# haoheliu/voicefixer

Hardware: AMD Instinct MI355X
Metric: seconds-of-44.1kHz-audio restored per wall-second (higher is better)
Workload: dtype f32

## Files before the change

include/vfx_hip.h:

```cpp
#ifndef VFX_HIP_H
#define VFX_HIP_H

#include <stddef.h>
#include <stdint.h>

#ifdef __cplusplus
extern "C" {
#endif

typedef void* vfx_stream_t;

#define VFX_OK 0
#define VFX_EINVAL (-1)
#define VFX_EALIGN (-2)
#define VFX_ERANGE (-3)
#define VFX_ENOTSUP (-4)

typedef struct {
    void* ptr;
    int64_t bstride, cstride, lstride;
    int64_t guard;
    const int32_t* rows;
} vfx_tensor;

// ... 22 lines not shown
    const float* w_direct;
    const float* w_wino4;
} vfx_act;

#define VFX_PAD_ZERO 0
#define VFX_PAD_REFLECT 1

int vfx_version(void);

const char* vfx_build_id(void);

uint64_t vfx_launch_count(void);

int vfx_last_conv_tile(void);


int vfx_conv1d_f32(const vfx_tensor* x, const float* w_packed, const float* bias,
                   const vfx_tensor* res, const vfx_tensor* y, int B, int Cin, int Cout, int L,
                   int k, int dilation, int pad_mode, const vfx_act* act, vfx_stream_t stream);

int vfx_conv1d_f16(const vfx_tensor* x, const void* w_f16, const float* bias, const vfx_tensor* res,
                   const vfx_tensor* y, int B, int C, int L, int dilation, const vfx_act* act, int32_t* range_flag,
                   vfx_stream_t stream);

typedef struct {
    const float* w1_direct;
    const float* bias1;
    const float* w2_direct;
    const float* bias2;
    const float* w2_wino;
// ... 147 lines not shown
```

voicefixer_amd/_lib.py:

```python
import ctypes as C
import os
import subprocess

from ._dev import dev_env

_HERE = os.path.dirname(os.path.abspath(__file__))
LIB_PATH = dev_env("VFX_LIB", os.path.join(_HERE, "libvfx_hip.so"))
CSRC = os.path.join(_HERE, "csrc")


class VfxError(RuntimeError):
    pass


class vfx_tensor(C.Structure):
    _fields_ = [("ptr", C.c_void_p), ("bstride", C.c_int64), ("cstride", C.c_int64),
                ("lstride", C.c_int64), ("guard", C.c_int64), ("rows", C.c_void_p)]


class vfx_act(C.Structure):
    _fields_ = [("pre_act", C.c_int), ("pre_slope", C.c_float), ("pre_scale", C.c_void_p),
                ("pre_shift", C.c_void_p), ("post_act", C.c_int), ("post_slope", C.c_float),
                ("math", C.c_int), ("w_x3", C.c_void_p), ("w_direct", C.c_void_p), ("w_wino4", C.c_void_p)]

# ... 7 lines not shown
POST_NONE, POST_LRELU, POST_ELU, POST_TANH, POST_SIGMOID, POST_LRELU_SNAKE = 0, 1, 2, 3, 4, 5
PAD_ZERO, PAD_REFLECT = 0, 1
MATH_F32, MATH_BF16X3 = 0, 1
EINVAL, EALIGN, ERANGE, ENOTSUP = -1, -2, -3, -4

_T = C.POINTER(vfx_tensor)
_A = C.POINTER(vfx_act)
_P = C.c_void_p
_I = C.c_int

SIGNATURES = {
    "vfx_version": (_I, []),
    "vfx_build_id": (C.c_char_p, []),
    "vfx_launch_count": (C.c_uint64, []),
    "vfx_last_conv_tile": (_I, []),
    "vfx_conv1d_f32": (_I, [_T, _P, _P, _T, _T, _I, _I, _I, _I, _I, _I, _I, _A, _P]),
    "vfx_conv1d_f16": (_I, [_T, _P, _P, _T, _T, _I, _I, _I, _I, _A, _P, _P]),
    "vfx_resblock_f32": (_I, [_T, _T, C.POINTER(vfx_resblock_w), _I, _I, _I, _I, C.c_float, _I, C.c_float, _P]),
    "vfx_resblock_wino4_f32": (_I, [_T, _T, C.POINTER(vfx_resblock_w), _I, _I, _I, _I, C.c_float, _I, C.c_float, _P]),
    "vfx_convtr1d_f32": (_I, [_T, _P, _P, _T, _I, _I, _I, _I, _I, _A, _P]),
    "vfx_conv2d_f32": (_I, [_T, _P, _P, _T, _T, _I, _I, _I, _I, _I, _I, _A, _P]),
    "vfx_convtr2d_3x3s2_f32": (_I, [_T, _P, _T, _I, _I, _I, _I, _I, _A, _P]),
    "vfx_conv1d_cout1_f32": (_I, [_T, _P, _P, _T, _I, _I, _I, _I, _I, _I, _I, _P]),
    "vfx_avgpool2x2_f32": (_I, [_T, _T, _I, _I, _I, _I, _P]),
    "vfx_frontend_init": (_I, [_P, _P, _P, _P, _P, _P, _I]),
    "vfx_frontend_readback": (_I, [_I, _P, _P, _P, _P, _I, C.POINTER(_I)]),
    "vfx_stft_mel_f32": (_I, [_P, C.c_int64, _I, _I, _P, _P]),
    "vfx_stft_mel_rows_f32": (_I, [_P, C.c_int64, _I, _P, _I, _P, _P]),
    "vfx_post_rows_f32": (_I, [_P, C.c_int64, _I, _P, _P, C.c_int64, _P, _I, _I, _P, _P]),
    "vfx_mel_to_cond_rows_f32": (_I, [_P, _T, _I, _I, _P, _I, _P]),
# ... 72 lines not shown
```

voicefixer_amd/csrc/vfx_conv.hip:

```cpp
#include "vfx_common.h"
#include <cstdio>
#include <cstdlib>
#include <cstring>
#include <map>
#include <mutex>
#include <string>
#include <type_traits>
#include <vector>

#ifndef VFX_X3_ABL
#define VFX_X3_ABL 0
#endif
#ifndef VFX_ABL
#define VFX_ABL 0
#endif
#define VFX_MAXPH 8
#define VFX_MAXT 9

typedef float f32x16 __attribute__((ext_vector_type(16)));
typedef unsigned int u32x4 __attribute__((ext_vector_type(4)));

#if VFX_ABL & 8
__device__ unsigned long long g_dbg[10];
__device__ unsigned long long g_dbgx[6];
// ... 942 lines not shown
            fprintf(stderr, "conv table:");
            const unsigned* w = reinterpret_cast<const unsigned*>(&tb);
            for (size_t i = 0; i < sizeof(PhaseTab) / 4; ++i) fprintf(stderr, " %08x", w[i]);
            fprintf(stderr, "\n");
        }
    }
    ConvTables* d = nullptr;
    if (hipMalloc((void**)&d, sizeof(ConvTables)) != hipSuccess) return nullptr;
    if (hipMemcpy(d, &tb, sizeof(ConvTables), hipMemcpyHostToDevice) != hipSuccess) return nullptr;
    cache.emplace(std::move(key), d);
    return d;
}

static thread_local int g_last_tile = 0;
extern "C" int vfx_last_conv_tile(void) { return g_last_tile; }

static inline int floor4(int v) { return v >= 0 ? (v & ~3) : -(((-v) + 3) & ~3); }

template <int BM, int BL, int WGM, int WGL, int KC, bool FAST, int NXV = 4, bool SPLITK = false>
static int launch_one(const ConvArgs& a, dim3 grid, size_t lds, hipStream_t s) {
    static unsigned long long attr_set = 0;
    int attr_dev = 0;
    if (hipGetDevice(&attr_dev) != hipSuccess) attr_dev = 0;
    auto kern = conv_taps_kernel<BM, BL, WGM, WGL, KC, FAST, NXV, SPLITK>;
    if (!((attr_set >> (attr_dev & 63)) & 1ull)) {
        hipError_t e = hipFuncSetAttribute(reinterpret_cast<const void*>(kern),
                                           hipFuncAttributeMaxDynamicSharedMemorySize, 160 * 1024);
        if (e != hipSuccess) return (int)e;
        attr_set |= 1ull << (attr_dev & 63);
    }
    {
        static const bool dump = VFX_DEV_ENV("VFX_DEBUG_ARGS") && atoi(VFX_DEV_ENV("VFX_DEBUG_ARGS")) != 0;
        if (dump) {
            fprintf(stderr, "conv_taps<%d,%d,%d,%d,%d,%d,%d,%d> grid %u %u %u lds %zu args:", BM, BL, WGM, WGL, KC, (int)FAST,
                    NXV, (int)SPLITK, grid.x, grid.y, grid.z, lds);
            const unsigned* w = reinterpret_cast<const unsigned*>(&a);
            for (size_t i = 0; i < sizeof(ConvArgs) / 4; ++i) fprintf(stderr, " %08x", w[i]);
            fprintf(stderr, "\n");
        }
    }
    hipLaunchKernelGGL(kern, grid, dim3(64 * WGM * WGL), lds, s, a);
    VFX_LAUNCHED();
    return vfx_last_error();
}

template <int BM, int BL, int WGM, int WGL, int KC>
static int launch_cfg(const ConvArgs& a, int ntiles, int gy, int gz, size_t lds, hipStream_t s) {
    const int nfast = a.tile_hi - a.tile_lo;
    int rc = VFX_OK;
    if (a.ksplit > 1) {
        if (nfast > 0) rc = launch_one<BM, BL, WGM, WGL, KC, true, 4, true>(a, dim3(nfast, gy, gz), lds, s);
        if (rc == VFX_OK && ntiles - nfast > 0)
            rc = launch_one<BM, BL, WGM, WGL, KC, false, 4, true>(a, dim3(ntiles - nfast, gy, gz), lds, s);
        return rc;
    }
    if (nfast > 0) {
        const dim3 grid((nfast + a.tpw - 1) / a.tpw, gy, gz);
// ... 98 lines not shown

template <int BM, int BL, int WGM, int WGL, int NT, int MODE, int ROWS = 1>
static int launch_x3_one(const ConvArgs& a, dim3 grid, size_t lds, hipStream_t s) {
    static unsigned long long attr_set = 0;
    int attr_dev = 0;
    if (hipGetDevice(&attr_dev) != hipSuccess) attr_dev = 0;
    auto kern = conv_x3_kernel<BM, BL, WGM, WGL, NT, MODE, ROWS>;
    if (!((attr_set >> (attr_dev & 63)) & 1ull)) {
        hipError_t e = hipFuncSetAttribute(reinterpret_cast<const void*>(kern),
                                           hipFuncAttributeMaxDynamicSharedMemorySize, 160 * 1024);
        if (e != hipSuccess) return (int)e;
        attr_set |= 1ull << (attr_dev & 63);
    }
    hipLaunchKernelGGL(kern, grid, dim3(256), lds, s, a);
    VFX_LAUNCHED();
    return vfx_last_error();
}

template <int BM, int BL, int WGM, int WGL>
static int launch_x3_tile(const ConvArgs& a, int nt, int mode, int rows, dim3 grid, size_t lds, hipStream_t s) {
    if (rows == 3 && nt == 3) return launch_x3_one<BM, BL, WGM, WGL, 3, 0, 3>(a, grid, lds, s);
    if (rows == 3) return launch_x3_one<BM, BL, WGM, WGL, 1, 0, 3>(a, grid, lds, s);
#define VFX_X3(NT_)                                                                                  \
    if (nt == NT_)                                                                                   \
        return mode == 2   ? launch_x3_one<BM, BL, WGM, WGL, NT_, 2>(a, grid, lds, s)                \
               : mode == 1 ? launch_x3_one<BM, BL, WGM, WGL, NT_, 1>(a, grid, lds, s)                \
                           : launch_x3_one<BM, BL, WGM, WGL, NT_, 0>(a, grid, lds, s);
    VFX_X3(1)
    VFX_X3(2)
    VFX_X3(3)
// ... 411 lines not shown
```

voicefixer_amd/csrc/vfx_convh.inc:

```

typedef _Float16 f16x8 __attribute__((ext_vector_type(8)));
typedef _Float16 f16x2 __attribute__((ext_vector_type(2)));
typedef float f32x2h __attribute__((ext_vector_type(2)));

namespace convh {
constexpr int BM = 128, BL = 128, KC = 32, NTHR = 256;
constexpr int NPMAX = 3 * BL;
constexpr int NU = (KC / 8) * NPMAX / NTHR;
constexpr int BUFB = (KC / 8) * NPMAX * 16;
constexpr float F16_MAX = 65504.f;
}

struct ConvhArgs {
    const float* x; long long x_bs, x_cs;
    const int32_t* x_rows;
    const _Float16* w;
    const float* bias;
    const float* res; long long r_bs, r_cs;
    float* y; long long y_bs, y_cs;
    int C, L, d, ntiles, nm;
    int pre_act; float pre_slope;
    int post_act; float post_slope;
    int32_t* flag;
};
// ... 162 lines not shown
    a.res = res ? static_cast<const float*>(res->ptr) : nullptr;
    a.r_bs = res ? res->bstride : 0; a.r_cs = res ? res->cstride : 0;
    a.y = static_cast<float*>(y->ptr); a.y_bs = y->bstride; a.y_cs = y->cstride;
    a.C = C; a.L = L; a.d = dilation;
    a.ntiles = (L + convh::BL - 1) / convh::BL;
    a.nm = C / convh::BM;
    a.pre_act = pre; a.pre_slope = act ? act->pre_slope : 0.f;
    a.post_act = post; a.post_slope = act ? act->post_slope : 0.f;
    a.flag = range_flag;
    const long long nblk = (long long)a.ntiles * a.nm;
    if (nblk > 0x7fffffffLL) return VFX_ENOTSUP;
    auto kern = bias ? (a.res ? convh_kernel<true, true> : convh_kernel<true, false>)
                     : (a.res ? convh_kernel<false, true> : convh_kernel<false, false>);
    hipLaunchKernelGGL(kern, dim3((unsigned)nblk, 1, B), dim3(convh::NTHR), 0, (hipStream_t)stream, a);
    VFX_LAUNCHED();
    g_last_tile = convh::BM * 100000 + convh::BL * 100 + 32;
    return vfx_last_error();
}
```

voicefixer_amd/csrc/vfx_convtw.inc:

```
template <int WGM, int WGP>
__global__ __launch_bounds__(256, 2) void convtw_kernel(const ConvArgs a) {
    static_assert(WGM * WGP == 4, "four waves");
    constexpr int KC = 16, NSTEP = KC / 2, NPL = 4;
    constexpr int BM = 32 * WGM, BT = 32 * WGP;
    constexpr int CG = 256 / BT;
    constexpr int NSLOT = KC / CG;
    constexpr int SPAN = NSTEP / NSLOT;
    constexpr int PLANE = KC * BT;
    constexpr int BUF = NPL * PLANE;
    extern __shared__ __attribute__((aligned(16))) float smem[];

    const int tid = threadIdx.x, lane = tid & 63;
    const int wave = __builtin_amdgcn_readfirstlane(tid >> 6);
    const int lo = lane & 31, hi = lane >> 5;
    const int wm = wave / WGP, wp = wave % WGP;
    const int s = a.nph_fold, gy = a.tpw;
    int lin = blockIdx.x;
    if (a.xcd_chunk > 0) lin = (lin & 7) * a.xcd_chunk + (lin >> 3);
    if (lin >= a.ntiles_l * gy) return;
    int mblk, tile;
    if (a.tile_lo == 0) {
        tile = lin % a.ntiles_l; mblk = lin / a.ntiles_l;
    } else {
        mblk = lin % gy; tile = lin / gy;
// ... 213 lines not shown
                for (int j = 0; j < 4; ++j) {
                    const bool one = !all4 && o4 + j >= 0 && o4 + j < sL;
                    __builtin_amdgcn_raw_buffer_store_b32(u[j], yrsrc, one ? yb + 4 * j : VFX_W_OOB, 0, 0);
                }
            }
        }
        __builtin_amdgcn_fence(__ATOMIC_ACQ_REL, "wavefront");
        __builtin_amdgcn_wave_barrier();
    }
}

template <int WGM, int WGP>
static int launch_convtw(const ConvArgs& a, dim3 grid, size_t lds, hipStream_t s) {
    hipLaunchKernelGGL((convtw_kernel<WGM, WGP>), grid, dim3(256), lds, s, a);
    VFX_LAUNCHED();
    return vfx_last_error();
}

static int try_launch_convtw(const vfx_tensor* x, const float* w_packed, const float* w32, const float* bias, const vfx_tensor* y, int B,
                             int Cin, int Cout, int Lin, int stride, const vfx_act* act, hipStream_t stream) {
    static const bool off = VFX_DEV_ENV("VFX_CONVTW") && atoi(VFX_DEV_ENV("VFX_CONVTW")) == 0;
    if (off || !w_packed || !w32 || !vfx_aligned16(w32) || !x || !y || !x->ptr || !y->ptr) return VFX_ENOTSUP;
    if (act && (act->pre_act != VFX_PRE_NONE || act->post_act != VFX_POST_NONE || act->math != VFX_MATH_F32)) return VFX_ENOTSUP;
    if (Cin < 32 || Cout <= 0 || Cin % 32 != 0 || Cout % 64 != 0 || B <= 0 || B > 65535 || Lin < 1 || stride < 1) return VFX_ENOTSUP;
    if (x->lstride != 1 || y->lstride != 1 || (bias && !vfx_aligned16(bias))) return VFX_ENOTSUP;
    const long long lim = (1ll << 31) - (1ll << 20);
    if (((long long)Cin * x->cstride + Lin) * 4 >= lim || ((long long)Cout * y->cstride + (long long)stride * Lin) * 4 >= lim) return VFX_ENOTSUP;
    if (4ll * stride * (Cin >> 3) * Cout * 32 >= lim || (long long)stride * stride * Cout >= (1ll << 32)) return VFX_ENOTSUP;
    const bool wide = Cout % 128 == 0;
    const int BT = wide ? 32 : 64;
// ... 30 lines not shown
```

voicefixer_amd/csrc/vfx_convw.inc:

```

#define VFX_W_MAXNT 3
#ifndef VFX_W_MULTITILE
#define VFX_W_MULTITILE 0
#endif

template <int RM>
struct WStream {
    int voff[RM];
    int gstride;
    int cin8;
    int slab0, slab_step;
    int nt;
    int t, c8, c8_last;
    float4 cur[RM], nxt[RM];

    __device__ __forceinline__ void load(__amdgpu_buffer_rsrc_t rsrc, float4 (&dst)[RM]) {
        const int soff = ((slab0 + t * slab_step) * cin8 + c8) * gstride;
#pragma unroll
        for (int i = 0; i < RM; ++i) {
            const u32x4 r = __builtin_amdgcn_raw_buffer_load_b128(rsrc, voff[i], soff, 0);
            dst[i] = make_float4(__uint_as_float(r.x), __uint_as_float(r.y), __uint_as_float(r.z), __uint_as_float(r.w));
        }
        int tn = t + 1, cn = c8;
        if (tn == nt) { tn = 0; cn = c8 + 1; }
// ... 793 lines not shown

template <int BM, int BL, int WGM, int WGL, int NT, int NXV, int FUSED>
static int launch_w_one(const ConvArgs& a, dim3 grid, size_t lds, hipStream_t s) {
    static unsigned long long attr_set = 0;
    int attr_dev = 0;
    if (hipGetDevice(&attr_dev) != hipSuccess) attr_dev = 0;
    auto kern = convw_kernel<BM, BL, WGM, WGL, NT, NXV, FUSED>;
    if (!((attr_set >> (attr_dev & 63)) & 1ull)) {
        hipError_t e = hipFuncSetAttribute(reinterpret_cast<const void*>(kern),
                                           hipFuncAttributeMaxDynamicSharedMemorySize, 160 * 1024);
        if (e != hipSuccess) return (int)e;
        attr_set |= 1ull << (attr_dev & 63);
    }
    hipLaunchKernelGGL(kern, grid, dim3(256), lds, s, a);
    VFX_LAUNCHED();
    return vfx_last_error();
}

template <int BM, int BL, int WGM, int WGL, int NT, int FUSED>
static int launch_w_nxv(const ConvArgs& a, dim3 grid, size_t lds, hipStream_t s) {
    if constexpr (FUSED) {
        return a.nxv <= 5 ? launch_w_one<BM, BL, WGM, WGL, NT, 5, FUSED>(a, grid, lds, s)
                          : launch_w_one<BM, BL, WGM, WGL, NT, 6, FUSED>(a, grid, lds, s);
    } else if constexpr (NT == 9) {
        return a.nxv <= 4 ? launch_w_one<BM, BL, WGM, WGL, NT, 4, false>(a, grid, lds, s)
                          : launch_w_one<BM, BL, WGM, WGL, NT, 7, false>(a, grid, lds, s);
    } else {
        return a.nxv <= 4   ? launch_w_one<BM, BL, WGM, WGL, NT, 4, false>(a, grid, lds, s)
               : a.nxv == 5 ? launch_w_one<BM, BL, WGM, WGL, NT, 5, false>(a, grid, lds, s)
                            : launch_w_one<BM, BL, WGM, WGL, NT, 6, false>(a, grid, lds, s);
// ... 320 lines not shown
```

voicefixer_amd/csrc/vfx_convwg.inc:

```

static void convwg_fold_blocks(ConvArgs& a, dim3& grid, int gy) {
    static const bool off = VFX_DEV_ENV("VFX_WINO_MFOLD") && atoi(VFX_DEV_ENV("VFX_WINO_MFOLD")) == 0;
    a.nph_fold = 0;
    if (gy > 1 && a.xcd_chunk > 0 && !off) {
        a.nph_fold = gy;
        grid = dim3(grid.x * gy, 1, grid.z);
    }
}

#ifndef VFX_WG4_OCC
#define VFX_WG4_OCC 2
#endif
#ifndef VFX_WG4_ABL
#define VFX_WG4_ABL 0
#endif
#ifndef VFX_WG4_SPEC2_OCC
#define VFX_WG4_SPEC2_OCC 2
#endif
template <int WGM, int WGP, bool D1 = false, int XD = 2, bool PRE = true, int SPEC = 0>
__global__ __launch_bounds__(256, (SPEC == 2 && WGM == 4) ? VFX_WG4_SPEC2_OCC : VFX_WG4_OCC) void convwg4_kernel(const ConvArgs a) {
    static_assert(WGM * WGP == 4, "four waves");
    static_assert(SPEC == 0 || (SPEC == 1 && PRE) || (SPEC == 2 && D1 && !PRE), "specialised instances");
    constexpr bool ZSTART = SPEC != 0;
    static_assert(XD == 2 || XD == 3, "prefetch distance");
// ... 494 lines not shown

template <int WGM, int WGP, bool D1 = false, int XD = 2, bool PRE = true, int SPEC = 0>
static int launch_wg4_xd(const ConvArgs& a, dim3 grid, size_t lds, hipStream_t s) {
    static unsigned long long attr_set = 0;
    int attr_dev = 0;
    if (hipGetDevice(&attr_dev) != hipSuccess) attr_dev = 0;
    auto kern = convwg4_kernel<WGM, WGP, D1, XD, PRE, SPEC>;
    if (!((attr_set >> (attr_dev & 63)) & 1ull)) {
        hipError_t e = hipFuncSetAttribute(reinterpret_cast<const void*>(kern),
                                           hipFuncAttributeMaxDynamicSharedMemorySize, 160 * 1024);
        if (e != hipSuccess) return (int)e;
        attr_set |= 1ull << (attr_dev & 63);
    }
    hipLaunchKernelGGL(kern, grid, dim3(256), lds, s, a);
    VFX_LAUNCHED();
    return vfx_last_error();
}

template <int WGM, int WGP, bool D1 = false>
static int launch_wg4_one(const ConvArgs& a, dim3 grid, size_t lds, hipStream_t s) {
#ifdef VFX_DEV
    static const int xd = VFX_DEV_ENV("VFX_WG4_XD") ? atoi(VFX_DEV_ENV("VFX_WG4_XD")) : 2;
    if (xd == 3) return launch_wg4_xd<WGM, WGP, D1, 3, true>(a, grid, lds, s);
    static const int spec_mask = VFX_DEV_ENV("VFX_WG4_SPEC") ? atoi(VFX_DEV_ENV("VFX_WG4_SPEC")) : 3;
#else
    constexpr int spec_mask = 3;
#endif
    if ((spec_mask & 1) && !a.res && a.pre_act == VFX_PRE_LRELU && a.post_act == VFX_POST_LRELU && (!a.bias || vfx_aligned16(a.bias)))
        return launch_wg4_xd<WGM, WGP, D1, 2, true, 1>(a, grid, lds, s);
    if constexpr (D1) {
// ... 84 lines not shown
```

voicefixer_amd/csrc/vfx_convwg2d.inc:

```
constexpr int WG4S_TWO_CIN = 384;
template <int WGM, int WGP, int KC, bool AFF = true, bool TWO = false>
__global__ __launch_bounds__(256, TWO ? 1 : 2) void convwg4s_kernel(const ConvArgs a) {
    static_assert(WGM * WGP == 4 && (KC == 8 || KC == 16), "four waves; 8- or 16-channel chunks");
    constexpr int NSTEP = KC / 2;
    constexpr int NG = KC / 8;
    constexpr int NSEQ = 3 * NG;
    constexpr int BM = 32 * WGM, BQ = 32 * WGP;
    constexpr int ROW = BQ + 2;
    constexpr int CG = 256 / BQ;
    constexpr int NSLOT = KC / CG;
    constexpr int PLANE = KC * ROW;
    constexpr int BUF = 6 * PLANE;
    static_assert(2 * NSLOT <= 3 * NSTEP, "two steps of staging per element must fit the chunk");
    extern __shared__ __attribute__((aligned(16))) float smem[];

    const int tid = threadIdx.x, lane = tid & 63;
    const int wave = __builtin_amdgcn_readfirstlane(tid >> 6);
    const int lo = lane & 31, hi = lane >> 5;
    const int wm = wave / WGP, wp = wave % WGP;
    int bx = blockIdx.x;
    int mblk = blockIdx.y;
    if (a.xcd_chunk > 0) {
        int k = bx >> 3;
        if (a.nph_fold > 1) {
// ... 272 lines not shown
                __builtin_amdgcn_raw_buffer_store_b32(__float_as_uint(keep ? fmaxf(y[i], y[i] * ps) : 0.f), yrsrc, yv[i], soff, 0);
        }
    } else {
#pragma unroll 1
        for (int r = 0; r < 16; ++r) {
            const int soff = (row0 + (r & 3) + 8 * (r >> 2)) * ycs4;
            float y[4];
            outs(r, y);
#pragma unroll
            for (int i = 0; i < 4; ++i)
                __builtin_amdgcn_raw_buffer_store_b32(__float_as_uint(keep ? vfx_post(y[i], post, ps) : 0.f), yrsrc, yv[i], soff, 0);
        }
    }
}

template <int WGM, int WGP, int KC, bool AFF, bool TWO>
static int launch_wg4s_aff(const ConvArgs& a, dim3 grid, size_t lds, hipStream_t s) {
    static unsigned long long attr_set = 0;
    int attr_dev = 0;
    if (hipGetDevice(&attr_dev) != hipSuccess) attr_dev = 0;
    auto kern = convwg4s_kernel<WGM, WGP, KC, AFF, TWO>;
    if (!((attr_set >> (attr_dev & 63)) & 1ull)) {
        hipError_t e = hipFuncSetAttribute(reinterpret_cast<const void*>(kern),
                                           hipFuncAttributeMaxDynamicSharedMemorySize, 160 * 1024);
        if (e != hipSuccess) return (int)e;
        attr_set |= 1ull << (attr_dev & 63);
    }
    hipLaunchKernelGGL(kern, grid, dim3(256), lds, s, a);
    VFX_LAUNCHED();
    return vfx_last_error();
}

template <int WGM, int WGP, int KC>
static int launch_wg4s_one(const ConvArgs& a, dim3 grid, size_t lds, hipStream_t s) {
    if (a.Cin > WG4S_TWO_CIN)
        return a.pre_act == VFX_PRE_NONE ? launch_wg4s_aff<WGM, WGP, KC, false, true>(a, grid, lds, s)
                                         : launch_wg4s_aff<WGM, WGP, KC, true, true>(a, grid, lds, s);
    return a.pre_act == VFX_PRE_NONE ? launch_wg4s_aff<WGM, WGP, KC, false, false>(a, grid, lds, s)
                                     : launch_wg4s_aff<WGM, WGP, KC, true, false>(a, grid, lds, s);
}

static int try_launch_convwg4s_2d(ConvArgs a, const vfx_tensor* x, int P, const float* wg4, hipStream_t stream) {
    static const bool off = (VFX_DEV_ENV("VFX_WINO") && atoi(VFX_DEV_ENV("VFX_WINO")) == 0) ||
                            (VFX_DEV_ENV("VFX_WINO4") && atoi(VFX_DEV_ENV("VFX_WINO4")) == 0) ||
// ... 17 lines not shown
            return VFX_ENOTSUP;
        if (18ll * (a.CinPad >> 3) * a.Cout * 32 >= lim) return VFX_ENOTSUP;
    }
    const int d = P;
    const long long nquads = ((long long)a.Lin + 4 * d - 1) / (4 * d) * d;
    const int ntiles = (int)((nquads + BQ - 1) / BQ);
    const int gy = a.Cout / (narrow ? 32 : 64);
    if ((long long)ntiles * gy * a.B < 384) return VFX_ENOTSUP;
    a.wd = wg4;
    a.wg_d = d;
    a.x_guard = 0;
    a.tab = nullptr;
    a.stagger = 0; a.stagger_wgs = 0;
    if (!a.res) { a.r_bs = a.x_bs; a.r_cs = a.x_cs; }
    const size_t lds = (2ull * 6 * kc * (BQ + 2) + 2ull * a.Cin) * sizeof(float);
    dim3 grid(convw_grid_x(a, ntiles), gy, a.B);
    convwg_fold_blocks(a, grid, gy);
    g_last_tile = (narrow ? 32 : 64) * 100000 + (4 * BQ % 1000) * 100 + 88;
    return narrow ? launch_wg4s_one<1, 4, 8>(a, grid, lds, stream) : launch_wg4s_one<2, 2, 16>(a, grid, lds, stream);
}
```

voicefixer_amd/csrc/vfx_convwg4p.inc:

```
template <int WGM, int WGP, bool D1, bool PRE, int SPEC>
__global__ __launch_bounds__(256, 2) void convwg4p_kernel(const ConvArgs a) {
    static_assert(WGM * WGP == 4, "four waves");
    static_assert((SPEC == 1 && PRE) || (SPEC == 2 && D1 && !PRE), "specialised instances only");
    constexpr int KC = 16, NSTEP = KC / 2;
    constexpr int BM = 32 * WGM, BQ = 32 * WGP;
    constexpr int CG = 256 / BQ;
    constexpr int NSLOT = KC / CG;
    constexpr int SPAN = NSTEP / NSLOT;
    constexpr int PLANE = KC * BQ;
    constexpr int BUF = 6 * PLANE;
    extern __shared__ __attribute__((aligned(16))) float smem[];

    const int tid = threadIdx.x, lane = tid & 63;
    const int wave = __builtin_amdgcn_readfirstlane(tid >> 6);
    const int lo = lane & 31, hi = lane >> 5;
    const int wm = wave / WGP, wp = wave % WGP;
    const int gy = a.nph_fold;
    const int per = gridDim.x >> 3;
    const int xcd = blockIdx.x & 7, jw = blockIdx.x >> 3;
    const int nend = min(a.B * a.ntiles_l * gy, (xcd + 1) * a.xcd_chunk);
    int n = xcd * a.xcd_chunk + jw;
    if (n >= nend) return;
    const int m0 = (jw % gy) * BM;
    const int d = D1 ? 1 : a.wg_d;
// ... 302 lines not shown

template <int WGM, int WGP, bool D1, bool PRE, int SPEC>
static int launch_wg4p(const ConvArgs& a, int nwg, size_t lds, hipStream_t s) {
    static unsigned long long attr_set = 0;
    int attr_dev = 0;
    if (hipGetDevice(&attr_dev) != hipSuccess) attr_dev = 0;
    auto kern = convwg4p_kernel<WGM, WGP, D1, PRE, SPEC>;
    if (!((attr_set >> (attr_dev & 63)) & 1ull)) {
        hipError_t e = hipFuncSetAttribute(reinterpret_cast<const void*>(kern),
                                           hipFuncAttributeMaxDynamicSharedMemorySize, 160 * 1024);
        if (e != hipSuccess) return (int)e;
        attr_set |= 1ull << (attr_dev & 63);
    }
    hipLaunchKernelGGL(kern, dim3(nwg), dim3(256), lds, s, a);
    VFX_LAUNCHED();
    return vfx_last_error();
}

static int vfx_cu_count() {
    static int cus[64] = {0};
    int dev = 0;
    if (hipGetDevice(&dev) != hipSuccess) dev = 0;
    dev &= 63;
    if (!cus[dev]) {
        hipDeviceProp_t p;
        cus[dev] = (hipGetDeviceProperties(&p, dev) == hipSuccess && p.multiProcessorCount > 0) ? p.multiProcessorCount : 256;
    }
    return cus[dev];
}

// ... 27 lines not shown
```

voicefixer_amd/csrc/vfx_convwg4x.inc:

```
#ifndef VFX_WG4X_ABL
#define VFX_WG4X_ABL 0
#endif
template <bool D1, bool PRE, int SPEC>
__global__ __launch_bounds__(256, 1) void convwg4x_kernel(const ConvArgs a) {
    static_assert((SPEC == 1 && PRE) || (SPEC == 2 && D1 && !PRE), "specialised instances only");
    constexpr int KC = 8, NSTEP = KC / 2;
    constexpr int BM = 128, BQ = 64;
    constexpr int CG = 256 / BQ;
    constexpr int NSLOT = KC / CG;
    constexpr int SPAN = NSTEP / NSLOT;
    constexpr int PLANE = KC * BQ;
    constexpr int BUF = 6 * PLANE;
    constexpr int OBUF = 32 * 4 * BQ;
    constexpr int TPK = D1 ? 1 : 4;
    constexpr int NSL = NSTEP * TPK;
    constexpr int NUNIT = D1 ? 32 : 128;
    constexpr int NIT = NUNIT / NSL;
    static_assert(NIT * NSL == NUNIT && NIT == 8, "an iteration is valid or not as a whole");
    static_assert(SPAN == 2, "staging map");
    extern __shared__ __attribute__((aligned(16))) float smem[];

    const int tid = threadIdx.x, lane = tid & 63;
    const int wave = __builtin_amdgcn_readfirstlane(tid >> 6);
    const int lo = lane & 31, hi = lane >> 5;
// ... 354 lines not shown

template <bool D1, bool PRE, int SPEC>
static int launch_wg4x(const ConvArgs& a, int nwg, size_t lds, hipStream_t s) {
    static unsigned long long attr_set = 0;
    int attr_dev = 0;
    if (hipGetDevice(&attr_dev) != hipSuccess) attr_dev = 0;
    auto kern = convwg4x_kernel<D1, PRE, SPEC>;
    if (!((attr_set >> (attr_dev & 63)) & 1ull)) {
        hipError_t e = hipFuncSetAttribute(reinterpret_cast<const void*>(kern),
                                           hipFuncAttributeMaxDynamicSharedMemorySize, 160 * 1024);
        if (e != hipSuccess) return (int)e;
        attr_set |= 1ull << (attr_dev & 63);
    }
    hipLaunchKernelGGL(kern, dim3(nwg), dim3(256), lds, s, a);
    VFX_LAUNCHED();
    return vfx_last_error();
}

static int try_launch_convwg4x(ConvArgs a, long long nquads, bool d1vec, hipStream_t stream) {
    const int S = a.Cin / 8;
    if (S < 8 || (S & 1)) return VFX_ENOTSUP;
    if (a.Cout % 128 != 0) return VFX_ENOTSUP;
    if (a.bias && !vfx_aligned16(a.bias)) return VFX_ENOTSUP;
    const bool first = !a.res && a.pre_act == VFX_PRE_LRELU && a.post_act == VFX_POST_LRELU;
    const bool second = d1vec && a.res && a.pre_act == VFX_PRE_NONE && a.post_act == VFX_POST_NONE;
    if (!first && !second) return VFX_ENOTSUP;
    const int gy = a.Cout / 128;
    const int ntiles = (int)((nquads + 63) / 64);
    const long long N = (long long)a.B * ntiles * gy;
    if (N >= (1ll << 30)) return VFX_ENOTSUP;
// ... 13 lines not shown
```

voicefixer_amd/csrc/vfx_resblk4.inc:

```
template <bool STRIP>
__device__ __forceinline__ void resblk4_body(const ConvArgs& a) {
    constexpr int C = 64, KC = 16, NSTEP = KC / 2, S = C / KC;
    constexpr int BQ = 64, CG = 256 / BQ, NSLOT = KC / CG;
    constexpr int PLANE = KC * BQ, BUF = 6 * PLANE;
    static_assert(NSTEP / NSLOT == 2, "two k-pair steps per staged element");
    extern __shared__ __attribute__((aligned(16))) float smem[];

    const int tid = threadIdx.x, lane = tid & 63;
    const int wave = __builtin_amdgcn_readfirstlane(tid >> 6);
    const int lo = lane & 31, hi = lane >> 5;
    const int wm = wave & 1, wq = wave >> 1;
    int bx = blockIdx.x;
    if (a.xcd_chunk > 0) {
        bx = (bx & 7) * a.xcd_chunk + (bx >> 3);
        if (bx >= a.ntiles_l) return;
    }
    const int b = blockIdx.z;
    const int d = a.wg_d;
    const float inv_d = 1.0f / (float)d;
    const int Lrow = a.x_rows ? __builtin_amdgcn_readfirstlane(a.x_rows[b]) : a.Lin;
    const int xcs = (int)a.x_cs;
    const int q0 = STRIP ? 0 : bx * a.bl_step;
    const int nq1 = a.rb_nq1;
    const int pshift = STRIP ? a.rs_pshift : 6, P = 1 << pshift, W = P - 4;
// ... 440 lines not shown
    const int ntiles = (L + a.bl_step - 1) / a.bl_step;
    const size_t lds = (size_t)C * a.yp * sizeof(float);
    const dim3 grid(convw_grid_x(a, ntiles), 1, B);
    static unsigned long long attr_set = 0;
    int attr_dev = 0;
    if (hipGetDevice(&attr_dev) != hipSuccess) attr_dev = 0;
    if (!((attr_set >> (attr_dev & 63)) & 1ull)) {
        hipError_t e = hipFuncSetAttribute(reinterpret_cast<const void*>(resblk4_kernel), hipFuncAttributeMaxDynamicSharedMemorySize,
                                           160 * 1024);
        if (e != hipSuccess) return (int)e;
        attr_set |= 1ull << (attr_dev & 63);
    }
    g_last_tile = C * 100000 + 256 * 100 + 96;
    hipLaunchKernelGGL(resblk4_kernel, grid, dim3(256), lds, (hipStream_t)stream, a);
    VFX_LAUNCHED();
    return vfx_last_error();
}

extern "C" int vfx_resblock_f32(const vfx_tensor* x, const vfx_tensor* y, const vfx_resblock_w* w, int B, int C, int L,
                                int dilation, float slope, int post_act, float post_slope, vfx_stream_t stream) {
    if (!w) return VFX_EINVAL;
    static const bool off = (VFX_DEV_ENV("VFX_FUSE_WINO44") && atoi(VFX_DEV_ENV("VFX_FUSE_WINO44")) == 0) ||
                            (VFX_DEV_ENV("VFX_FUSE_WINO4") && atoi(VFX_DEV_ENV("VFX_FUSE_WINO4")) == 0) ||
                            (VFX_DEV_ENV("VFX_FUSE_WINO") && atoi(VFX_DEV_ENV("VFX_FUSE_WINO")) == 0);
    if (off || !resblk4_takes(dilation) || !resblk4_args_ok(x, y, w, B, C, L, dilation, slope, post_act, post_slope)) {
        return resblock_convw(x, y, w->w1_direct, w->bias1, w->w2_direct, w->bias2, w->w2_wino, w->w2_wino4, B, C, L, dilation, slope,
                              post_act, post_slope, stream);
    }
    return resblk4_launch(x, y, w, B, C, L, dilation, slope, post_act, post_slope, stream);
}
// ... 1 lines not shown
```

voicefixer_amd/csrc/vfx_resblk4s.inc:

```
__global__ __launch_bounds__(256, 2) void resblk4s_kernel(const ConvArgs a) { resblk4_body<true>(a); }

extern "C" int vfx_resblock_wino4_f32(const vfx_tensor* x, const vfx_tensor* y, const vfx_resblock_w* w, int B, int C, int L,
                                      int dilation, float slope, int post_act, float post_slope, vfx_stream_t stream) {
    if (!w) return VFX_EINVAL;
    if (!resblk4_args_ok(x, y, w, B, C, L, dilation, slope, post_act, post_slope)) return VFX_ENOTSUP;
    if (resblk4_takes(dilation)) return resblk4_launch(x, y, w, B, C, L, dilation, slope, post_act, post_slope, stream);
    ConvArgs a;
    resblk4_fill_args(a, x, y, w, B, C, L, dilation, slope, post_act, post_slope);
    auto nseg_of = [&](int P) { return (dilation + P - 5) / (P - 4); };
    const int pshift = 32 * nseg_of(32) < 64 * nseg_of(64) ? 5 : 6;
    const int nseg = nseg_of(1 << pshift);
    a.rs_pshift = pshift;
    a.rs_nseg = nseg;
    const long long nblk = ((long long)L + 4ll * dilation - 1) / (4ll * dilation);
    const long long nsegs = nblk * nseg;
    const int G = 64 >> pshift;
    const long long ntiles = (nsegs + G - 1) / G;
    if (ntiles * G >= (1 << 20)) return VFX_ENOTSUP;
    const size_t lds = (size_t)C * a.yp * sizeof(float);
    const dim3 grid(convw_grid_x(a, (int)ntiles), 1, B);
    static unsigned long long attr_set = 0;
    int attr_dev = 0;
    if (hipGetDevice(&attr_dev) != hipSuccess) attr_dev = 0;
    if (!((attr_set >> (attr_dev & 63)) & 1ull)) {
        hipError_t e = hipFuncSetAttribute(reinterpret_cast<const void*>(resblk4s_kernel), hipFuncAttributeMaxDynamicSharedMemorySize,
                                           160 * 1024);
        if (e != hipSuccess) return (int)e;
        attr_set |= 1ull << (attr_dev & 63);
    }
    g_last_tile = C * 100000 + 256 * 100 + 97;
    hipLaunchKernelGGL(resblk4s_kernel, grid, dim3(256), lds, (hipStream_t)stream, a);
    VFX_LAUNCHED();
    return vfx_last_error();
}
```

Measured before the change: 1612.

## Add persistent Winograd-4 small-Cin conv kernel with cross-tile prefetch

Adds a persistent variant of the Winograd F(4,3) small-channel conv kernel. It launches about two workgroups per CU and partitions tiles into per-XCD chunks. Each workgroup walks its tiles and prefetches the next tile's inputs and first weight group during the last chunk of the current tile. This is meant to remove per-tile launch and prologue cost and overlap loads across tiles, at the cost of extra complexity and possible load imbalance. It also records the last grid size across all conv launchers for diagnostics.

New measurement: 1607. No clear change (-0.3%).

```diff
diff --git a/include/vfx_hip.h b/include/vfx_hip.h
--- a/include/vfx_hip.h
+++ b/include/vfx_hip.h
@@ -60,6 +60,8 @@
 
 int vfx_last_conv_tile(void);
 
+long long vfx_last_conv_grid(void);
+
 
 int vfx_conv1d_f32(const vfx_tensor* x, const float* w_packed, const float* bias,
                    const vfx_tensor* res, const vfx_tensor* y, int B, int Cin, int Cout, int L,
diff --git a/voicefixer_amd/_lib.py b/voicefixer_amd/_lib.py
--- a/voicefixer_amd/_lib.py
+++ b/voicefixer_amd/_lib.py
@@ -45,6 +45,7 @@
     "vfx_build_id": (C.c_char_p, []),
     "vfx_launch_count": (C.c_uint64, []),
     "vfx_last_conv_tile": (_I, []),
+    "vfx_last_conv_grid": (C.c_longlong, []),
     "vfx_conv1d_f32": (_I, [_T, _P, _P, _T, _T, _I, _I, _I, _I, _I, _I, _I, _A, _P]),
     "vfx_conv1d_f16": (_I, [_T, _P, _P, _T, _T, _I, _I, _I, _I, _A, _P, _P]),
     "vfx_resblock_f32": (_I, [_T, _T, C.POINTER(vfx_resblock_w), _I, _I, _I, _I, C.c_float, _I, C.c_float, _P]),
diff --git a/voicefixer_amd/csrc/vfx_conv.hip b/voicefixer_amd/csrc/vfx_conv.hip
--- a/voicefixer_amd/csrc/vfx_conv.hip
+++ b/voicefixer_amd/csrc/vfx_conv.hip
@@ -980,6 +980,8 @@
 
 static thread_local int g_last_tile = 0;
 extern "C" int vfx_last_conv_tile(void) { return g_last_tile; }
+static thread_local long long g_last_grid = 0;
+extern "C" long long vfx_last_conv_grid(void) { return g_last_grid; }
 
 static inline int floor4(int v) { return v >= 0 ? (v & ~3) : -(((-v) + 3) & ~3); }
 
@@ -1007,6 +1009,7 @@
     }
     hipLaunchKernelGGL(kern, grid, dim3(64 * WGM * WGL), lds, s, a);
     VFX_LAUNCHED();
+    g_last_grid = (long long)grid.x * grid.y * grid.z;
     return vfx_last_error();
 }
 
@@ -1135,6 +1138,7 @@
     }
     hipLaunchKernelGGL(kern, grid, dim3(256), lds, s, a);
     VFX_LAUNCHED();
+    g_last_grid = (long long)grid.x * grid.y * grid.z;
     return vfx_last_error();
 }
 
diff --git a/voicefixer_amd/csrc/vfx_convh.inc b/voicefixer_amd/csrc/vfx_convh.inc
--- a/voicefixer_amd/csrc/vfx_convh.inc
+++ b/voicefixer_amd/csrc/vfx_convh.inc
@@ -200,6 +200,7 @@
                      : (a.res ? convh_kernel<false, true> : convh_kernel<false, false>);
     hipLaunchKernelGGL(kern, dim3((unsigned)nblk, 1, B), dim3(convh::NTHR), 0, (hipStream_t)stream, a);
     VFX_LAUNCHED();
+    g_last_grid = (long long)nblk * B;
     g_last_tile = convh::BM * 100000 + convh::BL * 100 + 32;
     return vfx_last_error();
 }
diff --git a/voicefixer_amd/csrc/vfx_convtw.inc b/voicefixer_amd/csrc/vfx_convtw.inc
--- a/voicefixer_amd/csrc/vfx_convtw.inc
+++ b/voicefixer_amd/csrc/vfx_convtw.inc
@@ -251,6 +251,7 @@
 static int launch_convtw(const ConvArgs& a, dim3 grid, size_t lds, hipStream_t s) {
     hipLaunchKernelGGL((convtw_kernel<WGM, WGP>), grid, dim3(256), lds, s, a);
     VFX_LAUNCHED();
+    g_last_grid = (long long)grid.x * grid.y * grid.z;
     return vfx_last_error();
 }
 
diff --git a/voicefixer_amd/csrc/vfx_convw.inc b/voicefixer_amd/csrc/vfx_convw.inc
--- a/voicefixer_amd/csrc/vfx_convw.inc
+++ b/voicefixer_amd/csrc/vfx_convw.inc
@@ -831,6 +831,7 @@
     }
     hipLaunchKernelGGL(kern, grid, dim3(256), lds, s, a);
     VFX_LAUNCHED();
+    g_last_grid = (long long)grid.x * grid.y * grid.z;
     return vfx_last_error();
 }
 
diff --git a/voicefixer_amd/csrc/vfx_convwg.inc b/voicefixer_amd/csrc/vfx_convwg.inc
--- a/voicefixer_amd/csrc/vfx_convwg.inc
+++ b/voicefixer_amd/csrc/vfx_convwg.inc
@@ -532,6 +532,7 @@
     }
     hipLaunchKernelGGL(kern, grid, dim3(256), lds, s, a);
     VFX_LAUNCHED();
+    g_last_grid = (long long)grid.x * grid.y * grid.z;
     return vfx_last_error();
 }
 
diff --git a/voicefixer_amd/csrc/vfx_convwg2d.inc b/voicefixer_amd/csrc/vfx_convwg2d.inc
--- a/voicefixer_amd/csrc/vfx_convwg2d.inc
+++ b/voicefixer_amd/csrc/vfx_convwg2d.inc
@@ -310,6 +310,317 @@
     }
 }
 
+template <int WGM, int WGP, int KC>
+__global__ __launch_bounds__(256, 2) void convwg4sp_kernel(const ConvArgs a) {
+    static_assert(WGM * WGP == 4 && (KC == 8 || KC == 16), "four waves; 8- or 16-channel chunks");
+    constexpr int NSTEP = KC / 2;
+    constexpr int NG = KC / 8;
+    constexpr int NSEQ = 3 * NG;
+    constexpr int BM = 32 * WGM, BQ = 32 * WGP;
+    constexpr int ROW = BQ + 2;
+    constexpr int CG = 256 / BQ;
+    constexpr int NSLOT = KC / CG;
+    constexpr int PLANE = KC * ROW;
+    constexpr int BUF = 6 * PLANE;
+    static_assert(2 * NSLOT <= 3 * NSTEP, "two steps of staging per element must fit the chunk");
+    extern __shared__ __attribute__((aligned(16))) float smem[];
+
+    const int tid = threadIdx.x, lane = tid & 63;
+    const int wave = __builtin_amdgcn_readfirstlane(tid >> 6);
+    const int lo = lane & 31, hi = lane >> 5;
+    const int wm = wave / WGP, wp = wave % WGP;
+    const int gy = a.nph_fold;
+    const int per = gridDim.x >> 3;
+    const int xcd = blockIdx.x & 7, jw = blockIdx.x >> 3;
+    const int nend = min(a.B * a.ntiles_l * gy, (xcd + 1) * a.xcd_chunk);
+    int n = xcd * a.xcd_chunk + jw;
+    if (n >= nend) return;
+    const int m0 = (jw % gy) * BM;
+    const int d = a.wg_d;
+    const int dsh = 31 - __builtin_clz(d);
+    const int xcs = (int)a.x_cs;
+    const int S = a.Cin / KC;
+    auto quad_q = [&](int Q) __attribute__((always_inline)) {
+        const int blk = Q >> dsh;
+        return (blk << (dsh + 2)) + (Q - (blk << dsh));
+    };
+    const int sq = tid % BQ, cg = tid / BQ;
+
+    int t_b = 0, t_Q0 = 0, t_Lrow = 0, u_b = 0, u_Q0 = 0, u_Lrow = 0;
+    bool t_valid = false, u_valid = false;
+    auto tile_uniform = [&](int nn, int& b_, int& Q0_, int& Lrow_, bool& valid_) __attribute__((always_inline)) {
+        valid_ = nn < nend;
+        const int u = (valid_ ? nn : n) / gy;
+        b_ = u / a.ntiles_l;
+        Q0_ = (u - b_ * a.ntiles_l) * BQ;
+        Lrow_ = a.x_rows ? __builtin_amdgcn_readfirstlane(a.x_rows[b_]) : a.Lin;
+        const int nblk = (Lrow_ + 4 * d - 1) >> (dsh + 2);
+        valid_ = valid_ && Q0_ < nblk * d;
+    };
+    int xvoff[6];
+    auto tile_thread = [&](int Q0_, int Lrow_, bool valid_) __attribute__((always_inline)) {
+        const int q = quad_q(Q0_ + sq);
+        const bool padcol = (q & a.in_mask) == a.in_mask;
+#pragma unroll
+        for (int j = 0; j < 6; ++j) {
+            const int p = q + (j - 1) * d;
+            xvoff[j] = (valid_ && p >= 0 && p < Lrow_ && !padcol) ? (cg * xcs + p) * 4 : VFX_W_OOB;
+        }
+    };
+    auto x_rsrc = [&](int b_) __attribute__((always_inline)) {
+        return __builtin_amdgcn_make_buffer_rsrc(const_cast<float*>(a.x) + (long long)b_ * a.x_bs, (short)0, 0x7fffffff, 0x00020000);
+    };
+    float* const biasl = smem + 2 * BUF;
+    {
+        if (tid < BM) biasl[tid] = a.bias ? a.bias[m0 + tid] : 0.f;
+        for (int r = tid; r < 2 * 6 * KC; r += 256) {
+            smem[r * ROW] = 0.f;
+            smem[r * ROW + ROW - 1] = 0.f;
+        }
+        __syncthreads();
+    }
+    float* const wbase = smem + cg * ROW + 1 + sq;
+
+    float xv[NSLOT][6];
+    auto x_load = [&](const __amdgpu_buffer_rsrc_t& rs, int chunk) __attribute__((always_inline)) {
+        const int s0 = chunk * KC * xcs * 4;
+#pragma unroll
+        for (int j = 0; j < NSLOT; ++j)
+#pragma unroll
+            for (int t = 0; t < 6; ++t)
+                xv[j][t] = __uint_as_float(__builtin_amdgcn_raw_buffer_load_b32(rs, xvoff[t], s0 + j * CG * xcs * 4, 0));
+    };
+    auto x_transform = [&](int j, float (&V)[6]) __attribute__((always_inline)) {
+        float e[6];
+#pragma unroll
+        for (int t = 0; t < 6; ++t) e[t] = xv[j][t];
+        const float s1 = fmaf(-4.f, e[2], e[4]), s2 = fmaf(-4.f, e[1], e[3]);
+        const float s3 = e[4] - e[2], s4 = e[3] - e[1];
+        V[0] = fmaf(4.f, e[0], fmaf(-5.f, e[2], e[4]));
+        V[1] = s1 + s2;
+        V[2] = s1 - s2;
+        V[3] = fmaf(2.f, s4, s3);
+        V[4] = fmaf(-2.f, s4, s3);
+        V[5] = fmaf(4.f, e[1], fmaf(-5.f, e[3], e[5]));
+    };
+
+    const __amdgpu_buffer_rsrc_t wrsrc =
+        __builtin_amdgcn_make_buffer_rsrc(const_cast<float*>(a.wd), (short)0, 0x7fffffff, 0x00020000);
+    const int row0 = m0 + wm * 32;
+    const int avoff = ((row0 + lo) * 8 + 4 * hi) * 4;
+    const int gstride = a.Cout * 32;
+    const int pstride = (a.CinPad >> 3) * gstride;
+    float4 aw[2][6];
+    auto a_load_one = [&](auto set_tag, int k, int goff) __attribute__((always_inline)) {
+        constexpr int SET = decltype(set_tag)::value;
+        const u32x4 r = __builtin_amdgcn_raw_buffer_load_b128(wrsrc, avoff, k * pstride + goff, 0);
+        aw[SET][k] = make_float4(__uint_as_float(r.x), __uint_as_float(r.y), __uint_as_float(r.z), __uint_as_float(r.w));
+    };
+    f32x16 acc[6];
+    const int boffs = hi * ROW + wp * 32 + lo;
+
+    auto mma_chunk = [&](auto par_tag, const __amdgpu_buffer_rsrc_t& rsl, const float* xs, float* wdst, int cld, int ccur, int cnext) __attribute__((always_inline)) {
+        constexpr int PAR = decltype(par_tag)::value;
+        const float* bp = xs + boffs;
+        float bf[6];
+#pragma unroll
+        for (int k = 0; k < 6; ++k) bf[k] = bp[k * PLANE];
+        const int xs0 = cld * KC * xcs * 4;
+        const int acur = NG * ccur * gstride, anext = NG * cnext * gstride;
+        float V[6];
+#pragma unroll
+        for (int kx = 0; kx < 3; ++kx) {
+#pragma unroll
+            for (int u = 0; u < NSTEP; ++u) {
+                const int s = kx * NSTEP + u;
+                const int el = s >> 1, ph = s & 1;
+                const int gs = kx * NG + (u >> 2);
+                const bool newgrp = (u & 3) == 0;
+                const int gn = gs + 1;
+                const int goff_next = gn < NSEQ ? (gn / NG) * 6 * pstride + (gn % NG) * gstride + acur : anext;
+                const bool last_step = kx == 2 && u == NSTEP - 1;
+                const int un = u + 1 < NSTEP ? u + 1 : 0, kxn = u + 1 < NSTEP ? kx : kx + 1;
+#pragma unroll
+                for (int k = 0; k < 6; ++k) {
+                    if (el < NSLOT) {
+                        if (ph == 0 && k == 0) x_transform(el, V);
+                        if (ph == 0) wdst[el * CG * ROW + k * PLANE] = V[k];
+                        if (ph == 1)
+                            xv[el][k] = __uint_as_float(__builtin_amdgcn_raw_buffer_load_b32(rsl, xvoff[k], xs0 + el * CG * xcs * 4, 0));
+                    }
+                    if (newgrp) {
+                        if (((gs + 1 + PAR * NSEQ) & 1) == 0) a_load_one(std::integral_constant<int, 0>{}, k, goff_next);
+                        else a_load_one(std::integral_constant<int, 1>{}, k, goff_next);
+                    }
+                    const float4 av4 = ((gs + PAR * NSEQ) & 1) ? aw[1][k] : aw[0][k];
+                    const int kk = u & 3;
+                    const float av = kk == 0 ? av4.x : (kk == 1 ? av4.y : (kk == 2 ? av4.z : av4.w));
+                    acc[k] = __builtin_amdgcn_mfma_f32_32x32x2f32(av, bf[k], acc[k], 0, 0, 0);
+                    if (!last_step) bf[k] = bp[k * PLANE + un * 2 * ROW + kxn];
+                    __builtin_amdgcn_sched_barrier(0);
+                }
+            }
+        }
+    };
+    using P0 = std::integral_constant<int, 0>;
+    using P1 = std::integral_constant<int, 1>;
+
+    const int ycs4 = (int)a.y_cs * 4, rcs4 = (int)a.r_cs * 4;
+    const int post = a.post_act;
+    const float ps = a.post_slope;
+    float rl[2][16];
+
+    tile_uniform(n, t_b, t_Q0, t_Lrow, t_valid);
+    bool restart = true;
+#pragma unroll 1
+    for (; n < nend; n += per) {
+        tile_uniform(n + per, u_b, u_Q0, u_Lrow, u_valid);
+        if (t_valid) {
+            __amdgpu_buffer_rsrc_t xrs = x_rsrc(t_b);
+            if (restart) {
+                tile_thread(t_Q0, t_Lrow, true);
+                x_load(xrs, 0);
+#pragma unroll
+                for (int k = 0; k < 6; ++k) a_load_one(P0{}, k, 0);
+                __builtin_amdgcn_sched_barrier(0);
+#pragma unroll
+                for (int j = 0; j < NSLOT; ++j) {
+                    float V[6];
+                    x_transform(j, V);
+#pragma unroll
+                    for (int k = 0; k < 6; ++k) wbase[j * CG * ROW + k * PLANE] = V[k];
+                }
+                x_load(xrs, 1);
+                __builtin_amdgcn_sched_barrier(0);
+                __syncthreads();
+            }
+#pragma unroll
+            for (int k = 0; k < 6; ++k)
+#pragma unroll
+                for (int r = 0; r < 16; ++r) acc[k][r] = 0.f;
+            auto res_issue = [&](auto slot_tag, int bt) __attribute__((always_inline)) {
+                constexpr int SL = decltype(slot_tag)::value;
+                const bool has_res = a.res != nullptr;
+                const __amdgpu_buffer_rsrc_t rrs = __builtin_amdgcn_make_buffer_rsrc(
+                    const_cast<float*>(has_res ? a.res : a.x) + (long long)t_b * a.r_bs, (short)0, 0x7fffffff, 0x00020000);
+                const int qe = quad_q(t_Q0 + wp * 32 + lo);
+#pragma unroll
+                for (int i = 0; i < 4; ++i) {
+                    const int rvo = (has_res && qe + i * d < t_Lrow) ? (4 * hi * (int)a.r_cs + qe + i * d) * 4 : VFX_W_OOB;
+#pragma unroll
+                    for (int e = 0; e < 4; ++e)
+                        rl[SL][4 * i + e] = __uint_as_float(__builtin_amdgcn_raw_buffer_load_b32(rrs, rvo, (row0 + e + 8 * bt) * rcs4, 0));
+                }
+            };
+#pragma unroll 1
+            for (int s = 0; s < S; s += 2) {
+                const bool last = s == S - 2;
+                if (last) {
+                    tile_thread(u_Q0, u_Lrow, u_valid);
+                    xrs = x_rsrc(u_b);
+                }
+                mma_chunk(P0{}, xrs, smem, wbase + BUF, last ? 0 : s + 2, s, s + 1);
+                __syncthreads();
+                mma_chunk(P1{}, xrs, smem + BUF, wbase, last ? 1 : s + 3, s + 1, last ? 0 : s + 2);
+                __syncthreads();
+            }
+
+            const __amdgpu_buffer_rsrc_t yrsrc = __builtin_amdgcn_make_buffer_rsrc(
+                a.y + (long long)t_b * a.y_bs, (short)0, 0x7fffffff, 0x00020000);
+            const int qe = quad_q(t_Q0 + wp * 32 + lo);
+            const bool keep = (qe & a.out_mask) != a.out_mask;
+            const float* const bp4 = biasl + wm * 32 + 4 * hi;
+            int yv[4];
+#pragma unroll
+            for (int i = 0; i < 4; ++i) yv[i] = qe + i * d < t_Lrow ? (4 * hi * (int)a.y_cs + qe + i * d) * 4 : VFX_W_OOB;
+            auto out_batch = [&](auto slot_tag, int bt, auto post_tag) __attribute__((always_inline)) {
+                constexpr int SL = decltype(slot_tag)::value;
+                constexpr int PT = decltype(post_tag)::value;
+                const float4 b4 = *reinterpret_cast<const float4*>(bp4 + 8 * bt);
+#pragma unroll
+                for (int e = 0; e < 4; ++e) {
+                    const int r = 4 * bt + e;
+                    const int soff = (row0 + e + 8 * bt) * ycs4;
+                    const float p12 = acc[1][r] + acc[2][r], m12 = acc[1][r] - acc[2][r];
+                    const float p34 = acc[3][r] + acc[4][r], m34 = acc[3][r] - acc[4][r];
+                    const float bb = e == 0 ? b4.x : (e == 1 ? b4.y : (e == 2 ? b4.z : b4.w));
+                    float y[4];
+                    y[0] = (((acc[0][r] + p12) + p34) + bb) + rl[SL][e];
+                    y[1] = (fmaf(2.f, m34, m12) + bb) + rl[SL][4 + e];
+                    y[2] = (fmaf(4.f, p34, p12) + bb) + rl[SL][8 + e];
+                    y[3] = ((fmaf(8.f, m34, m12) + acc[5][r]) + bb) + rl[SL][12 + e];
+#pragma unroll
+                    for (int i = 0; i < 4; ++i) {
+                        const float v = PT == 0 ? y[i] : (PT == 1 ? fmaxf(y[i], y[i] * ps) : vfx_post(y[i], post, ps));
+                        __builtin_amdgcn_raw_buffer_store_b32(__float_as_uint(keep ? v : 0.f), yrsrc, yv[i], soff, 0);
+                    }
+                }
+            };
+            auto epilogue = [&](auto post_tag) __attribute__((always_inline)) {
+                res_issue(P0{}, 0);
+                res_issue(P1{}, 1);
+                __builtin_amdgcn_sched_barrier(0);
+                out_batch(P0{}, 0, post_tag);
+                res_issue(P0{}, 2);
+                __builtin_amdgcn_sched_barrier(0);
+                out_batch(P1{}, 1, post_tag);
+                res_issue(P1{}, 3);
+                __builtin_amdgcn_sched_barrier(0);
+                out_batch(P0{}, 2, post_tag);
+                out_batch(P1{}, 3, post_tag);
+                __builtin_amdgcn_sched_barrier(0);
+            };
+            if (post == VFX_POST_NONE) epilogue(std::integral_constant<int, 0>{});
+            else if (post == VFX_POST_LRELU) epilogue(std::integral_constant<int, 1>{});
+            else epilogue(std::integral_constant<int, 2>{});
+            restart = !u_valid;
+        } else {
+            restart = true;
+        }
+        t_b = u_b; t_Q0 = u_Q0; t_Lrow = u_Lrow; t_valid = u_valid;
+    }
+}
+
+template <int WGM, int WGP, int KC>
+static int launch_wg4sp(const ConvArgs& a, int nwg, size_t lds, hipStream_t s) {
+    static unsigned long long attr_set = 0;
+    int attr_dev = 0;
+    if (hipGetDevice(&attr_dev) != hipSuccess) attr_dev = 0;
+    auto kern = convwg4sp_kernel<WGM, WGP, KC>;
+    if (!((attr_set >> (attr_dev & 63)) & 1ull)) {
+        hipError_t e = hipFuncSetAttribute(reinterpret_cast<const void*>(kern),
+                                           hipFuncAttributeMaxDynamicSharedMemorySize, 160 * 1024);
+        if (e != hipSuccess) return (int)e;
+        attr_set |= 1ull << (attr_dev & 63);
+    }
+    hipLaunchKernelGGL(kern, dim3(nwg), dim3(256), lds, s, a);
+    VFX_LAUNCHED();
+    g_last_grid = nwg;
+    return vfx_last_error();
+}
+
+constexpr int WG4SP_MIN_ITEMS = 3;
+constexpr int WG4SP_MAX_CHUNKS = 4;
+static int try_launch_convwg4sp(ConvArgs a, int ntiles, int gy, bool narrow, hipStream_t stream) {
+    static const bool off = VFX_DEV_ENV("VFX_WINO4S_PERSIST") && atoi(VFX_DEV_ENV("VFX_WINO4S_PERSIST")) == 0;
+    static const int min_items = VFX_DEV_ENV("VFX_WG4SP_MIN") ? atoi(VFX_DEV_ENV("VFX_WG4SP_MIN")) : WG4SP_MIN_ITEMS;
+    static const int max_chunks = VFX_DEV_ENV("VFX_WG4SP_MAXS") ? atoi(VFX_DEV_ENV("VFX_WG4SP_MAXS")) : WG4SP_MAX_CHUNKS;
+    const int kc = narrow ? 8 : 16, BQ = narrow ? 128 : 64, BM = narrow ? 32 : 64;
+    if (off || a.pre_act != VFX_PRE_NONE || a.Cin > WG4S_TWO_CIN || a.Cin / kc > max_chunks) return VFX_ENOTSUP;
+    const long long N = (long long)a.B * ntiles * gy;
+    if (N >= (1ll << 30)) return VFX_ENOTSUP;
+    int nwg = 2 * vfx_cu_count();
+    nwg -= nwg % (8 * gy);
+    if (nwg < 8 * gy || N < (long long)min_items * nwg) return VFX_ENOTSUP;
+    long long chunk = (N + 7) / 8;
+    chunk = (chunk + gy - 1) / gy * gy;
+    a.ntiles_l = ntiles;
+    a.nph_fold = gy;
+    a.xcd_chunk = (int)chunk;
+    const size_t lds = (2ull * 6 * kc * (BQ + 2) + BM) * sizeof(float);
+    return narrow ? launch_wg4sp<1, 4, 8>(a, nwg, lds, stream) : launch_wg4sp<2, 2, 16>(a, nwg, lds, stream);
+}
+
 template <int WGM, int WGP, int KC, bool AFF, bool TWO>
 static int launch_wg4s_aff(const ConvArgs& a, dim3 grid, size_t lds, hipStream_t s) {
     static unsigned long long attr_set = 0;
@@ -324,6 +635,7 @@
     }
     hipLaunchKernelGGL(kern, grid, dim3(256), lds, s, a);
     VFX_LAUNCHED();
+    g_last_grid = (long long)grid.x * grid.y * grid.z;
     return vfx_last_error();
 }
 
@@ -371,8 +683,12 @@
     a.stagger = 0; a.stagger_wgs = 0;
     if (!a.res) { a.r_bs = a.x_bs; a.r_cs = a.x_cs; }
     const size_t lds = (2ull * 6 * kc * (BQ + 2) + 2ull * a.Cin) * sizeof(float);
+    g_last_tile = (narrow ? 32 : 64) * 100000 + (4 * BQ % 1000) * 100 + 88;
+    {
+        const int rc = try_launch_convwg4sp(a, ntiles, gy, narrow, stream);
+        if (rc != VFX_ENOTSUP) return rc;
+    }
     dim3 grid(convw_grid_x(a, ntiles), gy, a.B);
     convwg_fold_blocks(a, grid, gy);
-    g_last_tile = (narrow ? 32 : 64) * 100000 + (4 * BQ % 1000) * 100 + 88;
     return narrow ? launch_wg4s_one<1, 4, 8>(a, grid, lds, stream) : launch_wg4s_one<2, 2, 16>(a, grid, lds, stream);
 }
diff --git a/voicefixer_amd/csrc/vfx_convwg4p.inc b/voicefixer_amd/csrc/vfx_convwg4p.inc
--- a/voicefixer_amd/csrc/vfx_convwg4p.inc
+++ b/voicefixer_amd/csrc/vfx_convwg4p.inc
@@ -340,6 +340,7 @@
     }
     hipLaunchKernelGGL(kern, dim3(nwg), dim3(256), lds, s, a);
     VFX_LAUNCHED();
+    g_last_grid = nwg;
     return vfx_last_error();
 }
 
diff --git a/voicefixer_amd/csrc/vfx_convwg4x.inc b/voicefixer_amd/csrc/vfx_convwg4x.inc
--- a/voicefixer_amd/csrc/vfx_convwg4x.inc
+++ b/voicefixer_amd/csrc/vfx_convwg4x.inc
@@ -392,6 +392,7 @@
     }
     hipLaunchKernelGGL(kern, dim3(nwg), dim3(256), lds, s, a);
     VFX_LAUNCHED();
+    g_last_grid = nwg;
     return vfx_last_error();
 }
 
diff --git a/voicefixer_amd/csrc/vfx_resblk4.inc b/voicefixer_amd/csrc/vfx_resblk4.inc
--- a/voicefixer_amd/csrc/vfx_resblk4.inc
+++ b/voicefixer_amd/csrc/vfx_resblk4.inc
@@ -478,6 +478,7 @@
     g_last_tile = C * 100000 + 256 * 100 + 96;
     hipLaunchKernelGGL(resblk4_kernel, grid, dim3(256), lds, (hipStream_t)stream, a);
     VFX_LAUNCHED();
+    g_last_grid = (long long)grid.x * grid.y * grid.z;
     return vfx_last_error();
 }
 
diff --git a/voicefixer_amd/csrc/vfx_resblk4s.inc b/voicefixer_amd/csrc/vfx_resblk4s.inc
--- a/voicefixer_amd/csrc/vfx_resblk4s.inc
+++ b/voicefixer_amd/csrc/vfx_resblk4s.inc
@@ -31,5 +31,6 @@
     g_last_tile = C * 100000 + 256 * 100 + 97;
     hipLaunchKernelGGL(resblk4s_kernel, grid, dim3(256), lds, (hipStream_t)stream, a);
     VFX_LAUNCHED();
+    g_last_grid = (long long)grid.x * grid.y * grid.z;
     return vfx_last_error();
 }
```
